# pananananas/MVD

Measured on AMD Instinct MI355X. Metric: UNet forward-passes/sec @512x512 SD2.1+MV adapter, higher is better.
Workload: dtype bf16; 1 GPU; cfg4: configs[3]/[4]: 8 objects x 4 target views per GPU (32 pairs), camera FiLM + cross-view adapter; pairs_per_gpu=32, global_pairs=32, latent=64x64x4, image=512x512, forward=cold, hip_graph=False, q2_statistics=replica-local, parallelism=dp1 (pairs sharded by object), weights=synthetic seeded, SD2.1 shapes (865.9M UNet x2 + 99.2M adapter + 19.1M camera), encoder_weights=distinct

## Files before the change

### include/mvd_hip.h

```cpp
#ifndef MVD_HIP_H
#define MVD_HIP_H
#include <stddef.h>
#include <stdint.h>

#ifdef __cplusplus
extern "C" {
#endif

#define MVD_MAX_LEVELS 4

typedef struct {
  int in_channels;
  int out_channels;
  int num_levels;
  int block_out_channels[MVD_MAX_LEVELS];
  int num_heads[MVD_MAX_LEVELS];
  int layers_per_block;
  int cross_attention_dim;
  int norm_num_groups;
  float norm_eps;
  int cam_output_dim;
  int cam_hidden_dim;
  int simple_cam_encoder;
  float cam_modulation_strength;
// ... 109 lines not shown
int mvd_op_refnorm(const void* x, int batch, int hw, int c, void* y, void* stream);
int mvd_op_refnorm_grouped(const void* x, int batch, int group, int hw, int c, void* y, void* stream);
int mvd_op_film(const void* x, int batch, int hw, int c, const float* scale, const float* shift, void* y, void* stream);
int mvd_op_conv_in(const void* x, int batch, int h, int w, int cin, const float* wt, const float* bias, int cout, void* y,
                   void* stream);
int mvd_op_conv_out(const void* x, int batch, int h, int w, int c, const void* wt, const float* bias, int cout, float* y,
                    void* stream);
int mvd_op_nchw_to_nhwc(const float* x, int batch, int c, int hw, const float* scale, const float* shift, void* y,
                        void* stream);
int mvd_op_nhwc_to_nchw(const void* x, int batch, int hw, int c, float* y, void* stream);
int mvd_op_f32_to_bf16(const float* x, int64_t n, void* y, void* stream);
int mvd_op_skinny_linear(const float* x, int ldx, int batch, int k, const void* w, int wbf16, const float* bias, int n, int act_in,
                         float* y, int ldy, void* stream);
int mvd_gemm_num_configs(void);
int mvd_debug_last_gemm_plan(int* out);
int mvd_debug_last_attention_plan(int* out);
int mvd_debug_last_groupnorm_plan(int* out);
long mvd_debug_up4_launches(void);
int mvd_debug_last_gemm_nowait(void);
int mvd_debug_pick_splitk(int m, int n, int k, int geglu);
int mvd_debug_pick_splitk_conv(int m, int n, int k);
int mvd_gemm_sm_num_tiles(void);
int mvd_debug_set_attention_nw(int nw_log2);
int mvd_debug_ragged_tables(const int* view_counts, int objects, int g, int* adapter, int* text);
int mvd_debug_attention_mapped_grouped(const void* q, const void* k, const void* v, void* o, int batch, int heads, int nq, int nk,
                                       int ldq, int ldk, int ldv, int ldo, float scale, int kv_group, int kv_objects,
                                       const int* kv_index_host, int kv_elements, void* stream);
typedef enum {
  MVD_DBG_NO_SM_LN_FOLD = 1,
  MVD_DBG_SM_NO_SPLITK = 2,
  MVD_DBG_NO_SM = 4,
  MVD_DBG_NO_SPLIT_KV = 8,
  MVD_DBG_ONE_STREAM = 16,
  MVD_DBG_SINGLE_STREAM_POLICY = 32,
  MVD_DBG_SIDE_DEFAULT_PRIORITY = 64,
  MVD_DBG_NO_XS = 128,
  MVD_DBG_NO_WS = 256,
  MVD_DBG_WS_SMALL_MAPS = 512,
  MVD_DBG_WS_BLOCK64 = 1024,
  MVD_DBG_WS_NO_SHORTCUT = 2048,
  MVD_DBG_WS_NOT_IN_ENCODER = 4096,
  MVD_DBG_WS_ONLY_IN_ENCODER = 8192,
  MVD_DBG_WS_THEN_TILED = 16384,
  MVD_DBG_WS_CHECK = 32768,
  MVD_DBG_GRAPH_ONE_STREAM = 65536,
  MVD_DBG_PP_ROW_MAJOR = 131072,
  MVD_DBG_NO_DEEP_CONV_SPLIT = 262144,
  MVD_DBG_LATE_FROM_UP1 = 524288,
  MVD_DBG_NO_UP4 = 1048576,
  MVD_DBG_GN_ONE_PASS = 2097152,
  MVD_DBG_FORK_LATE = 4194304,
  MVD_DBG_SKINNY_VECTOR = 8388608
} mvd_debug_flag_t;
int mvd_debug_set_flags(int flags);

int mvd_op_ddpm_step(const float* model_out, const float* sample, const float* noise, float c0, float c1, float c2,
                     float c3, float sigma, float* out, int64_t n, void* stream);
int mvd_op_cfg_combine(const float* uncond_cond, float guidance_scale, float* out, int64_t n_half, void* stream);
int mvd_op_sampler_step(const float* model_out, int guided, float guidance_scale, const float* sample, const float* x0_prev,
                        const float* noise, float a0, float a1, float p, float q, float r, float sigma, float* out,
                        float* x0_out, int64_t n, void* stream);
int mvd_op_cfg_rescale(const float* uncond_cond, float guidance_scale, float guidance_rescale, float* out, int64_t rows,
                       int64_t n_row, void* stream);
int mvd_op_sampler_step_rescaled(const float* model_out, float guidance_scale, float guidance_rescale, const float* sample,
                                 const float* x0_prev, const float* noise, float a0, float a1, float p, float q, float r,
                                 float sigma, float* out, float* x0_out, int64_t rows, int64_t n_row, void* stream);
int mvd_debug_cfg_rescale_plan(int64_t n_row, int* out);

int mvd_op_freeu(const void* hidden, int C, const void* skip, int Cs, int B, int H, int W, float b, float s, void* hidden_out,
                 void* skip_out, void* stream);

int mvd_op_add_noise(const float* x0, const float* noise, const int32_t* timesteps, const float* sqrt_ac, const float* sqrt_1mac,
                     int num_train_timesteps, float* noisy, float* velocity, int batch, int64_t per_sample, void* stream);
int64_t mvd_op_noise_loss_ws_bytes(int batch, int64_t per_sample);
int mvd_op_noise_loss(const float* pred, const float* noise, const float* x0, const float* noisy, const int32_t* timesteps,
                      const float* sqrt_ac, const float* sqrt_1mac, const float* snr, int num_train_timesteps, int prediction_type,
                      float snr_gamma, float* denoised, float* result, int batch, int64_t per_sample, void* ws, int64_t ws_bytes,
                      void* stream);
int64_t mvd_op_image_metrics_ws_bytes(int n, int c, int h, int w, int want_ssim);
int mvd_op_image_metrics(const float* x, const float* y, int n, int c, int h, int w, float data_range, int want_ssim, float* result,
                         float* per_image, void* ws, int64_t ws_bytes, void* stream);

typedef struct {
  int in_channels;
  int latent_channels;
  int num_levels;
  int block_out_channels[MVD_MAX_LEVELS];
  int layers_per_block;
  int norm_num_groups;
  float norm_eps;
} mvd_vae_config_t;
typedef struct mvd_vae mvd_vae_t;
int mvd_vae_create(const mvd_vae_config_t* cfg, mvd_vae_t** out);
int mvd_vae_destroy(mvd_vae_t* v);
int mvd_vae_set_weight(mvd_vae_t* v, const char* slot, const void* ptr, int64_t numel, int dtype);
int64_t mvd_vae_workspace_bytes(mvd_vae_t* v, int batch, int height, int width, int decode);
int mvd_vae_bind_workspace(mvd_vae_t* v, void* ws, int64_t ws_bytes);
int mvd_vae_encode(mvd_vae_t* v, const float* image_nchw, int batch, int height, int width, float* moments, void* stream);
int mvd_vae_decode(mvd_vae_t* v, const float* latents_nchw, int batch, int height, int width, float* image, void* stream);
int64_t mvd_vae_mid_attention_workspace_bytes(mvd_vae_t* v, int decoder, int batch, int height, int width);
int mvd_vae_mid_attention(mvd_vae_t* v, int decoder, const void* x_nhwc_bf16, int batch, int height, int width, void* out_nhwc_bf16,
                          void* stream);
int mvd_op_softmax_rows(const float* s, int rows, int n, void* p_bf16, void* stream);
int mvd_op_gaussian_sample(const float* moments, const float* noise, int batch, int channels, int hw, float scale, float* out,
                           void* stream);

typedef struct {
// ... 120 lines not shown
```

### mvd_amd/_lib.py

```python
from __future__ import annotations

import ctypes as C
import enum
import os

HERE = os.path.dirname(os.path.abspath(__file__))
LIB_PATH = os.environ.get("MVD_HIP_LIB") or os.path.join(HERE, "libmvd_hip.so")

MVD_MAX_LEVELS = 4
MVD_USE_CAMERA, MVD_USE_IMAGE, MVD_REUSE_REF, MVD_KEEP_FEATURES, MVD_SHARE_REF = 1, 2, 4, 8, 16


class MvdError(RuntimeError):
    pass


class DebugFlag(enum.IntFlag):
    NO_SM_LN_FOLD = 1
    SM_NO_SPLITK = 2
    NO_SM = 4
    NO_SPLIT_KV = 8
    ONE_STREAM = 16
    SINGLE_STREAM_POLICY = 32
    SIDE_DEFAULT_PRIORITY = 64
    NO_XS = 128
    NO_WS = 256
    WS_SMALL_MAPS = 512
    WS_BLOCK64 = 1024
    WS_NO_SHORTCUT = 2048
    WS_NOT_IN_ENCODER = 4096
    WS_ONLY_IN_ENCODER = 8192
    WS_THEN_TILED = 16384
    WS_CHECK = 32768
    GRAPH_ONE_STREAM = 65536
    PP_ROW_MAJOR = 131072
    NO_DEEP_CONV_SPLIT = 262144
    LATE_FROM_UP1 = 524288
    NO_UP4 = 1048576
    GN_ONE_PASS = 2097152
    FORK_LATE = 4194304
    SKINNY_VECTOR = 8388608


class mvd_config_t(C.Structure):
    _fields_ = [
        ("in_channels", C.c_int), ("out_channels", C.c_int), ("num_levels", C.c_int),
        ("block_out_channels", C.c_int * MVD_MAX_LEVELS), ("num_heads", C.c_int * MVD_MAX_LEVELS),
        ("layers_per_block", C.c_int), ("cross_attention_dim", C.c_int), ("norm_num_groups", C.c_int),
        ("norm_eps", C.c_float), ("cam_output_dim", C.c_int), ("cam_hidden_dim", C.c_int),
        ("simple_cam_encoder", C.c_int), ("cam_modulation_strength", C.c_float),
    ]


class mvd_vae_config_t(C.Structure):
    _fields_ = [
        ("in_channels", C.c_int), ("latent_channels", C.c_int), ("num_levels", C.c_int),
        ("block_out_channels", C.c_int * MVD_MAX_LEVELS), ("layers_per_block", C.c_int), ("norm_num_groups", C.c_int),
        ("norm_eps", C.c_float),
    ]


class mvd_text_config_t(C.Structure):
    _fields_ = [
        ("vocab_size", C.c_int), ("hidden_size", C.c_int), ("intermediate_size", C.c_int), ("num_layers", C.c_int),
        ("num_heads", C.c_int), ("max_positions", C.c_int), ("layer_norm_eps", C.c_float), ("act", C.c_int),
    ]


class mvd_vision_config_t(C.Structure):
    _fields_ = [
        ("image_size", C.c_int), ("patch_size", C.c_int), ("hidden_size", C.c_int), ("intermediate_size", C.c_int),
        ("num_layers", C.c_int), ("num_heads", C.c_int), ("projection_dim", C.c_int), ("layer_norm_eps", C.c_float), ("act", C.c_int),
    ]


class mvd_forward_args_t(C.Structure):
    _fields_ = [
        ("batch", C.c_int), ("height", C.c_int), ("width", C.c_int), ("text_len", C.c_int),
        ("sample", C.c_void_p), ("timesteps", C.c_void_p), ("text", C.c_void_p),
        ("source_camera", C.c_void_p), ("target_camera", C.c_void_p), ("cam_rows", C.c_int), ("cam_batch", C.c_int),
        ("fourier_proj", C.c_void_p), ("source_latents", C.c_void_p), ("encoder_text", C.c_void_p),
        ("ref_batch", C.c_int), ("flags", C.c_int), ("out", C.c_void_p), ("views", C.c_int),
    ]


_SIGS = {
    "mvd_last_error": (C.c_char_p, []),
    "mvd_engine_create": (C.c_int, [C.POINTER(mvd_config_t), C.POINTER(C.c_void_p)]),
    "mvd_engine_destroy": (C.c_int, [C.c_void_p]),
    "mvd_engine_set_weight": (C.c_int, [C.c_void_p, C.c_int, C.c_char_p, C.c_void_p, C.c_int64, C.c_int]),
    "mvd_engine_clear_weights": (C.c_int, [C.c_void_p, C.c_int]),
    "mvd_engine_workspace_bytes": (C.c_int64, [C.c_void_p, C.c_int, C.c_int, C.c_int, C.c_int, C.c_int]),
    "mvd_engine_workspace_bytes_args": (C.c_int64, [C.c_void_p, C.POINTER(mvd_forward_args_t)]),
    "mvd_engine_workspace_bytes_objects": (C.c_int64, [C.c_void_p, C.POINTER(mvd_forward_args_t), C.c_int]),
# ... 21 lines not shown
    "mvd_engine_get_camera_embedding": (C.c_int, [C.c_void_p, C.c_void_p, C.c_void_p]),
    "mvd_op_linear": (C.c_int, [C.c_void_p, C.c_void_p, C.c_int, C.c_int, C.c_void_p, C.c_void_p, C.c_void_p, C.c_int,
                                C.c_int, C.c_void_p, C.c_float, C.c_int, C.c_void_p, C.c_int, C.c_int, C.c_int, C.c_int,
                                C.c_int, C.c_void_p, C.c_void_p]),
    "mvd_op_ln_linear": (C.c_int, [C.c_void_p, C.c_int, C.c_void_p, C.c_void_p, C.c_void_p, C.c_float, C.c_int, C.c_void_p,
                                   C.c_int, C.c_int, C.c_void_p]),
    "mvd_op_linear_xs": (C.c_int, [C.c_void_p, C.c_int, C.c_void_p, C.c_int, C.c_int, C.c_int, C.c_int, C.c_int, C.c_float,
                                   C.c_void_p, C.c_int, C.c_void_p, C.c_int, C.c_int, C.c_void_p]),
    "mvd_op_conv3x3_ws": (C.c_int, [C.c_void_p, C.c_int, C.c_int, C.c_int, C.c_int, C.c_void_p, C.c_void_p, C.c_void_p, C.c_int,
                                    C.c_void_p, C.c_void_p, C.c_void_p, C.c_int, C.c_int, C.c_void_p, C.c_int, C.c_int, C.c_void_p]),
    "mvd_op_conv3x3": (C.c_int, [C.c_void_p, C.c_int, C.c_int, C.c_int, C.c_int, C.c_int, C.c_int, C.c_int, C.c_void_p, C.c_void_p,
                                 C.c_void_p, C.c_int, C.c_void_p, C.c_void_p, C.c_void_p, C.c_int, C.c_int, C.c_void_p,
                                 C.c_int, C.c_int, C.c_int, C.c_void_p, C.c_void_p]),
    "mvd_op_attention": (C.c_int, [C.c_void_p, C.c_void_p, C.c_void_p, C.c_void_p, C.c_int, C.c_int, C.c_int, C.c_int,
                                   C.c_int, C.c_int, C.c_int, C.c_int, C.c_float, C.c_void_p]),
    "mvd_op_attention_grouped": (C.c_int, [C.c_void_p, C.c_void_p, C.c_void_p, C.c_void_p, C.c_int, C.c_int, C.c_int, C.c_int,
                                           C.c_int, C.c_int, C.c_int, C.c_int, C.c_float, C.c_int, C.c_void_p]),
    "mvd_op_attention_objects": (C.c_int, [C.c_void_p, C.c_void_p, C.c_void_p, C.c_void_p, C.c_int, C.c_int, C.c_int, C.c_int,
                                           C.c_int, C.c_int, C.c_int, C.c_int, C.c_float, C.c_int, C.c_int, C.c_void_p]),
    "mvd_op_attention_mapped": (C.c_int, [C.c_void_p, C.c_void_p, C.c_void_p, C.c_void_p, C.c_int, C.c_int, C.c_int, C.c_int,
                                          C.c_int, C.c_int, C.c_int, C.c_int, C.c_float, C.POINTER(C.c_int), C.c_int, C.c_void_p]),
    "mvd_debug_attention_mapped_grouped": (C.c_int, [C.c_void_p, C.c_void_p, C.c_void_p, C.c_void_p, C.c_int, C.c_int, C.c_int, C.c_int,
                                                     C.c_int, C.c_int, C.c_int, C.c_int, C.c_float, C.c_int, C.c_int, C.POINTER(C.c_int),
                                                     C.c_int, C.c_void_p]),
    "mvd_op_attention_split_ws_bytes": (C.c_int64, [C.c_int, C.c_int, C.c_int, C.c_int]),
    "mvd_op_attention_split": (C.c_int, [C.c_void_p, C.c_void_p, C.c_void_p, C.c_void_p, C.c_int, C.c_int, C.c_int, C.c_int, C.c_int,
                                         C.c_int, C.c_int, C.c_int, C.c_int, C.c_void_p, C.c_void_p]),
    "mvd_op_groupnorm": (C.c_int, [C.c_void_p, C.c_void_p, C.c_int, C.c_int, C.c_int, C.c_int, C.c_int, C.c_float,
                                   C.c_void_p, C.c_void_p, C.c_int, C.c_void_p, C.c_void_p, C.c_void_p]),
    "mvd_op_layernorm": (C.c_int, [C.c_void_p, C.c_int, C.c_int, C.c_float, C.c_void_p, C.c_void_p, C.c_void_p, C.c_void_p]),
    "mvd_op_refnorm": (C.c_int, [C.c_void_p, C.c_int, C.c_int, C.c_int, C.c_void_p, C.c_void_p]),
    "mvd_op_refnorm_grouped": (C.c_int, [C.c_void_p, C.c_int, C.c_int, C.c_int, C.c_int, C.c_void_p, C.c_void_p]),
    "mvd_op_film": (C.c_int, [C.c_void_p, C.c_int, C.c_int, C.c_int, C.c_void_p, C.c_void_p, C.c_void_p, C.c_void_p]),
    "mvd_op_conv_in": (C.c_int, [C.c_void_p, C.c_int, C.c_int, C.c_int, C.c_int, C.c_void_p, C.c_void_p, C.c_int, C.c_void_p, C.c_void_p]),
    "mvd_op_conv_out": (C.c_int, [C.c_void_p, C.c_int, C.c_int, C.c_int, C.c_int, C.c_void_p, C.c_void_p, C.c_int, C.c_void_p, C.c_void_p]),
    "mvd_op_nchw_to_nhwc": (C.c_int, [C.c_void_p, C.c_int, C.c_int, C.c_int, C.c_void_p, C.c_void_p, C.c_void_p, C.c_void_p]),
    "mvd_op_nhwc_to_nchw": (C.c_int, [C.c_void_p, C.c_int, C.c_int, C.c_int, C.c_void_p, C.c_void_p]),
    "mvd_op_f32_to_bf16": (C.c_int, [C.c_void_p, C.c_int64, C.c_void_p, C.c_void_p]),
    "mvd_op_skinny_linear": (C.c_int, [C.c_void_p, C.c_int, C.c_int, C.c_int, C.c_void_p, C.c_int, C.c_void_p, C.c_int, C.c_int,
                                        C.c_void_p, C.c_int, C.c_void_p]),
    "mvd_gemm_num_configs": (C.c_int, []),
    "mvd_debug_last_gemm_plan": (C.c_int, [C.POINTER(C.c_int)]),
    "mvd_debug_up4_launches": (C.c_long, []),
    "mvd_op_conv3x3_up4": (C.c_int, [C.c_void_p, C.c_int, C.c_int, C.c_int, C.c_int, C.c_void_p, C.c_void_p, C.c_void_p, C.c_int, C.c_int,
                                     C.c_void_p]),
    "mvd_debug_last_gemm_nowait": (C.c_int, []),
    "mvd_debug_last_attention_plan": (C.c_int, [C.POINTER(C.c_int)]),
    "mvd_debug_last_groupnorm_plan": (C.c_int, [C.POINTER(C.c_int)]),
    "mvd_debug_pick_splitk": (C.c_int, [C.c_int, C.c_int, C.c_int, C.c_int]),
    "mvd_debug_pick_splitk_conv": (C.c_int, [C.c_int, C.c_int, C.c_int]),
    "mvd_gemm_sm_num_tiles": (C.c_int, []),
    "mvd_debug_set_attention_nw": (C.c_int, [C.c_int]),
    "mvd_debug_set_flags": (C.c_int, [C.c_int]),
    "mvd_op_ddpm_step": (C.c_int, [C.c_void_p, C.c_void_p, C.c_void_p, C.c_float, C.c_float, C.c_float, C.c_float,
                                   C.c_float, C.c_void_p, C.c_int64, C.c_void_p]),
    "mvd_op_cfg_combine": (C.c_int, [C.c_void_p, C.c_float, C.c_void_p, C.c_int64, C.c_void_p]),
    "mvd_op_sampler_step": (C.c_int, [C.c_void_p, C.c_int, C.c_float, C.c_void_p, C.c_void_p, C.c_void_p, C.c_float, C.c_float,
                                      C.c_float, C.c_float, C.c_float, C.c_float, C.c_void_p, C.c_void_p, C.c_int64, C.c_void_p]),
    "mvd_op_cfg_rescale": (C.c_int, [C.c_void_p, C.c_float, C.c_float, C.c_void_p, C.c_int64, C.c_int64, C.c_void_p]),
    "mvd_op_sampler_step_rescaled": (C.c_int, [C.c_void_p, C.c_float, C.c_float, C.c_void_p, C.c_void_p, C.c_void_p, C.c_float,
                                               C.c_float, C.c_float, C.c_float, C.c_float, C.c_float, C.c_void_p, C.c_void_p,
                                               C.c_int64, C.c_int64, C.c_void_p]),
    "mvd_debug_cfg_rescale_plan": (C.c_int, [C.c_int64, C.POINTER(C.c_int)]),
    "mvd_engine_set_freeu": (C.c_int, [C.c_void_p, C.c_float, C.c_float, C.c_float, C.c_float]),
    "mvd_engine_clear_freeu": (C.c_int, [C.c_void_p]),
    "mvd_op_freeu": (C.c_int, [C.c_void_p, C.c_int, C.c_void_p, C.c_int, C.c_int, C.c_int, C.c_int, C.c_float, C.c_float, C.c_void_p,
                               C.c_void_p, C.c_void_p]),
    "mvd_op_add_noise": (C.c_int, [C.c_void_p, C.c_void_p, C.c_void_p, C.c_void_p, C.c_void_p, C.c_int, C.c_void_p, C.c_void_p, C.c_int,
                                   C.c_int64, C.c_void_p]),
    "mvd_op_noise_loss_ws_bytes": (C.c_int64, [C.c_int, C.c_int64]),
    "mvd_op_noise_loss": (C.c_int, [C.c_void_p, C.c_void_p, C.c_void_p, C.c_void_p, C.c_void_p, C.c_void_p, C.c_void_p, C.c_void_p,
                                    C.c_int, C.c_int, C.c_float, C.c_void_p, C.c_void_p, C.c_int, C.c_int64, C.c_void_p, C.c_int64,
                                    C.c_void_p]),
    "mvd_op_image_metrics_ws_bytes": (C.c_int64, [C.c_int, C.c_int, C.c_int, C.c_int, C.c_int]),
    "mvd_op_image_metrics": (C.c_int, [C.c_void_p, C.c_void_p, C.c_int, C.c_int, C.c_int, C.c_int, C.c_float, C.c_int, C.c_void_p,
                                       C.c_void_p, C.c_void_p, C.c_int64, C.c_void_p]),
    "mvd_vae_create": (C.c_int, [C.POINTER(mvd_vae_config_t), C.POINTER(C.c_void_p)]),
    "mvd_vae_destroy": (C.c_int, [C.c_void_p]),
    "mvd_vae_set_weight": (C.c_int, [C.c_void_p, C.c_char_p, C.c_void_p, C.c_int64, C.c_int]),
    "mvd_vae_workspace_bytes": (C.c_int64, [C.c_void_p, C.c_int, C.c_int, C.c_int, C.c_int]),
    "mvd_vae_bind_workspace": (C.c_int, [C.c_void_p, C.c_void_p, C.c_int64]),
    "mvd_vae_encode": (C.c_int, [C.c_void_p, C.c_void_p, C.c_int, C.c_int, C.c_int, C.c_void_p, C.c_void_p]),
    "mvd_vae_decode": (C.c_int, [C.c_void_p, C.c_void_p, C.c_int, C.c_int, C.c_int, C.c_void_p, C.c_void_p]),
    "mvd_vae_mid_attention_workspace_bytes": (C.c_int64, [C.c_void_p, C.c_int, C.c_int, C.c_int, C.c_int]),
    "mvd_vae_mid_attention": (C.c_int, [C.c_void_p, C.c_int, C.c_void_p, C.c_int, C.c_int, C.c_int, C.c_void_p, C.c_void_p]),
    "mvd_op_softmax_rows": (C.c_int, [C.c_void_p, C.c_int, C.c_int, C.c_void_p, C.c_void_p]),
    "mvd_op_gaussian_sample": (C.c_int, [C.c_void_p, C.c_void_p, C.c_int, C.c_int, C.c_int, C.c_float, C.c_void_p, C.c_void_p]),
    "mvd_text_create": (C.c_int, [C.POINTER(mvd_text_config_t), C.POINTER(C.c_void_p)]),
    "mvd_text_destroy": (C.c_int, [C.c_void_p]),
    "mvd_text_set_weight": (C.c_int, [C.c_void_p, C.c_char_p, C.c_void_p, C.c_int64, C.c_int]),
    "mvd_text_workspace_bytes": (C.c_int64, [C.c_void_p, C.c_int, C.c_int]),
    "mvd_text_bind_workspace": (C.c_int, [C.c_void_p, C.c_void_p, C.c_int64]),
    "mvd_text_encode": (C.c_int, [C.c_void_p, C.c_void_p, C.c_int, C.c_int, C.c_void_p, C.c_void_p]),
    "mvd_op_attention_causal": (C.c_int, [C.c_void_p, C.c_void_p, C.c_void_p, C.c_void_p, C.c_int, C.c_int, C.c_int, C.c_int,
                                          C.c_int, C.c_int, C.c_int, C.c_float, C.c_void_p]),
    "mvd_vision_create": (C.c_int, [C.POINTER(mvd_vision_config_t), C.POINTER(C.c_void_p)]),
    "mvd_vision_destroy": (C.c_int, [C.c_void_p]),
    "mvd_vision_set_weight": (C.c_int, [C.c_void_p, C.c_char_p, C.c_void_p, C.c_int64, C.c_int]),
    "mvd_vision_workspace_bytes": (C.c_int64, [C.c_void_p, C.c_int, C.c_int, C.c_int, C.c_int]),
    "mvd_vision_bind_workspace": (C.c_int, [C.c_void_p, C.c_void_p, C.c_int64]),
    "mvd_vision_preprocess": (C.c_int, [C.c_void_p, C.c_void_p, C.c_int, C.c_int, C.c_int, C.c_int, C.c_int, C.c_int,
                                        C.POINTER(C.c_float), C.POINTER(C.c_float), C.c_int, C.c_void_p, C.c_void_p]),
    "mvd_vision_patch_rows_offset": (C.c_int64, [C.c_void_p]),
    "mvd_vision_encode": (C.c_int, [C.c_void_p, C.c_void_p, C.c_int, C.c_void_p, C.c_void_p, C.c_void_p, C.c_void_p]),
    "mvd_op_clip_pool_project": (C.c_int, [C.c_void_p, C.c_void_p, C.c_void_p, C.c_int, C.c_int, C.c_int, C.c_int, C.c_void_p,
                                           C.c_void_p, C.c_float, C.c_void_p, C.c_int, C.c_void_p, C.c_void_p, C.c_void_p]),
# ... 146 lines not shown
```

### mvd_amd/csrc/misc.hip

```cpp
#include <stdarg.h>
#include <stdio.h>
#include <stdlib.h>
#include "host_util.h"

static thread_local char g_err[512] = "";
void mvd_set_error(const char* fmt, ...) {
  va_list ap;
  va_start(ap, fmt);
  vsnprintf(g_err, sizeof(g_err), fmt, ap);
  va_end(ap);
}
extern "C" const char* mvd_last_error(void) { return g_err; }

namespace {

__global__ void nchw_to_nhwc_kernel(const float* __restrict__ x, int c, int hw, const float* __restrict__ scale,
                                    const float* __restrict__ shift, int ld_ss, bf16_t* __restrict__ y, long total) {
  const long i = (long)blockIdx.x * blockDim.x + threadIdx.x;
  if (i >= total) return;
  const int ch = i % c;
  const long bp = i / c;
  const int p = bp % hw;
  const int b = bp / hw;
  float v = x[((size_t)b * c + ch) * hw + p];
  if (scale) v = v * scale[(size_t)b * ld_ss + ch] + shift[(size_t)b * ld_ss + ch];
  y[i] = f2bf(v);
}

__global__ void nhwc_to_nchw_f32_kernel(const bf16_t* __restrict__ x, int hw, int c, float* __restrict__ y, long total) {
  const long i = (long)blockIdx.x * blockDim.x + threadIdx.x;
  if (i >= total) return;
  const int p = i % hw;
  const long bc = i / hw;
  const int ch = bc % c;
  const int b = bc / c;
  y[i] = bf2f(x[((size_t)b * hw + p) * c + ch]);
}

__global__ void film_kernel(const bf16_t* __restrict__ x, int hw, int c, const float* __restrict__ scale,
                            const float* __restrict__ shift, int ld_ss, bf16_t* __restrict__ y, long nvec) {
  const int vec = c >> 3;
  for (long e = (long)blockIdx.x * blockDim.x + threadIdx.x; e < nvec; e += (long)gridDim.x * blockDim.x) {
    const int v = e % vec;
    const long bp = e / vec;
    const int b = bp / hw;
    const u32x4 in = *reinterpret_cast<const u32x4*>(x + e * 8);
    const float* sc = scale + (size_t)b * ld_ss + v * 8;
    const float* sf = shift + (size_t)b * ld_ss + v * 8;
    u32x4 o;
#pragma unroll
    for (int j = 0; j < 4; ++j)
      o[j] = pack2bf(fmaf(bflo(in[j]), sc[2 * j], sf[2 * j]), fmaf(bfhi(in[j]), sc[2 * j + 1], sf[2 * j + 1]));
    *reinterpret_cast<u32x4*>(y + e * 8) = o;
  }
}

__global__ void conv_in_kernel(const bf16_t* __restrict__ x, int h, int w, int cin, const float* __restrict__ wt,
                               const float* __restrict__ bias, int cout, bf16_t* __restrict__ y, long total) {
// ... 10 lines not shown
#pragma unroll
  for (int j = 0; j < 8; ++j) acc[j] = bias[g * 8 + j];
  for (int tap = 0; tap < 9; ++tap) {
    const int iy = oy + tap / 3 - 1, ix = ox + tap % 3 - 1;
    if ((unsigned)iy >= (unsigned)h || (unsigned)ix >= (unsigned)w) continue;
    const bf16_t* xp = x + ((size_t)b * hw + iy * w + ix) * cin;
    for (int ci = 0; ci < cin; ++ci) {
      const float xv = bf2f(xp[ci]);
#pragma unroll
      for (int j = 0; j < 8; ++j) acc[j] = fmaf(xv, wt[((size_t)(g * 8 + j) * 9 + tap) * cin + ci], acc[j]);
    }
  }
  u32x4 o = {pack2bf(acc[0], acc[1]), pack2bf(acc[2], acc[3]), pack2bf(acc[4], acc[5]), pack2bf(acc[6], acc[7])};
  *reinterpret_cast<u32x4*>(y + bp * cout + g * 8) = o;
}

__global__ __launch_bounds__(256) void conv_out_kernel(const bf16_t* __restrict__ x, int batch, int h, int w, int c,
                                                        const bf16_t* __restrict__ wt, const float* __restrict__ bias,
                                                        int cout, float* __restrict__ y) {
  const int lane = threadIdx.x & 63;
  const long pix = (long)blockIdx.x * 4 + (threadIdx.x >> 6);
  const int hw = h * w;
  if (pix >= (long)batch * hw) return;
  const int b = pix / hw, p = pix % hw;
  const int oy = p / w, ox = p % w;
  const int vec = c >> 3;
  float acc[8];
#pragma unroll
  for (int j = 0; j < 8; ++j) acc[j] = 0.f;
  for (int q = lane; q < 9 * vec; q += 64) {
    const int tap = q / vec, v = q % vec;
    const int iy = oy + tap / 3 - 1, ix = ox + tap % 3 - 1;
    if ((unsigned)iy >= (unsigned)h || (unsigned)ix >= (unsigned)w) continue;
    const u32x4 xv = *reinterpret_cast<const u32x4*>(x + ((size_t)b * hw + iy * w + ix) * c + v * 8);
#pragma unroll
    for (int co = 0; co < 8; ++co) {
      if (co < cout) {
        const u32x4 wv = *reinterpret_cast<const u32x4*>(wt + ((size_t)co * 9 + tap) * c + v * 8);
        float a = acc[co];
#pragma unroll
        for (int j = 0; j < 4; ++j) {
          a = fmaf(bflo(xv[j]), bflo(wv[j]), a);
          a = fmaf(bfhi(xv[j]), bfhi(wv[j]), a);
        }
        acc[co] = a;
      }
    }
  }
#pragma unroll
  for (int co = 0; co < 8; ++co) {
    if (co < cout) {
      const float t = wave_sum(acc[co]);
      if (lane == 0) y[((size_t)b * cout + co) * hw + p] = t + bias[co];
    }
  }
}

__global__ void f32_to_bf16_kernel(const float* __restrict__ x, long n, bf16_t* __restrict__ y) {
  for (long i = (long)blockIdx.x * blockDim.x + threadIdx.x; i < n; i += (long)gridDim.x * blockDim.x) y[i] = f2bf(x[i]);
}

template <bool WBF16>
__global__ __launch_bounds__(256) void skinny_linear_kernel(const float* __restrict__ x, int ldx, int batch, int k,
                                                             const void* __restrict__ wv, const float* __restrict__ bias,
                                                             int n, int act_in, float* __restrict__ y, int ldy) {
  constexpr int BC = 32;
  const int lane = threadIdx.x & 63;
  const int o = blockIdx.x * 4 + (threadIdx.x >> 6);
  if (o >= n) return;
  const bool vec = !WBF16 && (k & 3) == 0 && (ldx & 3) == 0;
  for (int b0 = 0; b0 < batch; b0 += BC) {
    float acc[BC];
#pragma unroll
    for (int j = 0; j < BC; ++j) acc[j] = 0.f;
    if (vec) {
      const float* wr = reinterpret_cast<const float*>(wv) + (size_t)o * k;
      for (int kk = lane * 4; kk < k; kk += 256) {
        const f32x4 w4 = *reinterpret_cast<const f32x4*>(wr + kk);
#pragma unroll
        for (int j = 0; j < BC; ++j) {
          if (b0 + j < batch) {
            f32x4 x4 = *reinterpret_cast<const f32x4*>(x + (size_t)(b0 + j) * ldx + kk);
            if (act_in == 1) { x4[0] = silu_f(x4[0]); x4[1] = silu_f(x4[1]); x4[2] = silu_f(x4[2]); x4[3] = silu_f(x4[3]); }
            acc[j] = fmaf(x4[0], w4[0], fmaf(x4[1], w4[1], fmaf(x4[2], w4[2], fmaf(x4[3], w4[3], acc[j]))));
          }
        }
      }
    } else {
      for (int kk = lane; kk < k; kk += 64) {
        float wgt;
        if (WBF16) wgt = bf2f(reinterpret_cast<const bf16_t*>(wv)[(size_t)o * k + kk]);
        else wgt = reinterpret_cast<const float*>(wv)[(size_t)o * k + kk];
#pragma unroll
        for (int j = 0; j < BC; ++j) {
          if (b0 + j < batch) {
            float xv = x[(size_t)(b0 + j) * ldx + kk];
            if (act_in == 1) xv = silu_f(xv);
            acc[j] = fmaf(xv, wgt, acc[j]);
          }
        }
      }
    }
#pragma unroll
    for (int j = 0; j < BC; ++j) {
      if (b0 + j < batch) {
        const float t = wave_sum(acc[j]);
// ... 279 lines not shown
  for (long i = (long)blockIdx.x * blockDim.x + threadIdx.x; i < n; i += (long)gridDim.x * blockDim.x) {
    const float va = a[i], vb = b[i], vr = r[i];
    if (__float_as_uint(va) != __float_as_uint(vb)) { __hip_atomic_fetch_add(cnt, 1ull, __ATOMIC_RELAXED, __HIP_MEMORY_SCOPE_SYSTEM); __hip_atomic_store(cnt + 3, (unsigned long long)i, __ATOMIC_RELAXED, __HIP_MEMORY_SCOPE_SYSTEM); }
    if (!(fabsf(va - vr) <= tol)) __hip_atomic_fetch_add(cnt + 1, 1ull, __ATOMIC_RELAXED, __HIP_MEMORY_SCOPE_SYSTEM);
    if (!(fabsf(vb - vr) <= tol)) __hip_atomic_fetch_add(cnt + 2, 1ull, __ATOMIC_RELAXED, __HIP_MEMORY_SCOPE_SYSTEM);
  }
}
#endif

int mvd_launch_conv_out(const bf16_t* x, int batch, int h, int w, int c, const bf16_t* wt, const float* bias, int cout,
                        float* y, hipStream_t s) {
  if (!x || !y || !wt || !bias || batch <= 0 || h <= 0 || w <= 0 || (c % 8) || cout <= 0 || cout > 8) { mvd_set_error("conv_out: bad arguments"); return -1; }
#ifdef MVD_PROBE
  if (MVD_ENV_INT("MVD_CONV_OUT4", 0)) {
    const long quads = (long)batch * h * ((w + 3) / 4);
    hipLaunchKernelGGL(conv_out4_kernel, dim3(nblk(quads, 4)), dim3(256), 0, s, x, batch, h, w, c, wt, bias, cout, y);
    if (MVD_ENV_INT("MVD_CONV_OUT_HASH", 0)) {
      static unsigned long long* dsum = nullptr; static float* y1 = nullptr; static size_t y1n = 0;
      const size_t on = (size_t)batch * cout * h * w;
      if (!dsum) (void)hipMalloc(&dsum, 3 * sizeof(unsigned long long));
      if (y1n < on) { if (y1) (void)hipFree(y1); (void)hipMalloc(&y1, on * sizeof(float)); y1n = on; }
      (void)hipMemsetAsync(dsum, 0, 3 * sizeof(unsigned long long), s);
      const long pix1 = (long)batch * h * w;
      hipLaunchKernelGGL(conv_out_kernel, dim3(nblk(pix1, 4)), dim3(256), 0, s, x, batch, h, w, c, wt, bias, cout, y1);
      hipLaunchKernelGGL(word_sum_kernel, dim3(1024), dim3(256), 0, s, reinterpret_cast<const unsigned*>(x), (long)((size_t)batch * h * w * c / 2), dsum);
      hipLaunchKernelGGL(word_sum_kernel, dim3(1024), dim3(256), 0, s, reinterpret_cast<const unsigned*>(y), (long)on, dsum + 1);
      hipLaunchKernelGGL(word_sum_kernel, dim3(1024), dim3(256), 0, s, reinterpret_cast<const unsigned*>(y1), (long)on, dsum + 2);
      unsigned long long hs[3] = {0, 0, 0};
      (void)hipMemcpyAsync(hs, dsum, sizeof(hs), hipMemcpyDeviceToHost, s);
      (void)hipStreamSynchronize(s);
      fprintf(stderr, "conv_out hash pid %d: input %016llx  out(4-pixel) %016llx  out(1-pixel, same input) %016llx\n", (int)getpid(), hs[0], hs[1], hs[2]);
    }
    if (MVD_ENV_INT("MVD_CONV_OUT_CMP", 0)) {
      static unsigned long long* cnt = nullptr; static float* yb = nullptr; static float* yr = nullptr; static size_t yn = 0;
      static unsigned long long seen[3] = {0, 0, 0}; static int calls = 0;
      const size_t on = (size_t)batch * cout * h * w;
      if (!cnt) { (void)hipHostMalloc(&cnt, 4 * sizeof(unsigned long long), hipHostMallocMapped); cnt[0] = cnt[1] = cnt[2] = cnt[3] = 0; }
      if (yn < on) { if (yb) { (void)hipFree(yb); (void)hipFree(yr); } (void)hipMalloc(&yb, on * sizeof(float)); (void)hipMalloc(&yr, on * sizeof(float)); yn = on; }
      hipLaunchKernelGGL(conv_out4_kernel, dim3(nblk(quads, 4)), dim3(256), 0, s, x, batch, h, w, c, wt, bias, cout, yb);
      hipLaunchKernelGGL(conv_out_kernel, dim3(nblk((long)batch * h * w, 4)), dim3(256), 0, s, x, batch, h, w, c, wt, bias, cout, yr);
      hipLaunchKernelGGL(conv_out_cmp_kernel, dim3(256), dim3(256), 0, s, y, yb, yr, (long)on, 1e-3f, cnt);
      ++calls;
      volatile unsigned long long* vc = cnt;
      const unsigned long long c0 = vc[0], c1 = vc[1], c2 = vc[2];
      if (c0 != seen[0] || c1 != seen[1] || c2 != seen[2] || calls == 2 || calls == 20) {
        seen[0] = c0; seen[1] = c1; seen[2] = c2;
        fprintf(stderr, "conv_out cmp pid %d after ~%d calls: first!=second %llu  |first-ref|>1e-3 %llu  |second-ref|>1e-3 %llu  last idx %llu (x mod 4 = %llu)\n",
                (int)getpid(), calls - 1, c0, c1, c2, (unsigned long long)vc[3], (unsigned long long)vc[3] % 4);
      }
    }
    return launch_check("conv_out4");
  }
#endif
  const long pix = (long)batch * h * w;
  hipLaunchKernelGGL(conv_out_kernel, dim3(nblk(pix, 4)), dim3(256), 0, s, x, batch, h, w, c, wt, bias, cout, y);
  return launch_check("conv_out");
}

int mvd_launch_f32_to_bf16(const float* x, int64_t n, bf16_t* y, hipStream_t s) {
  if (!x || !y || n <= 0) { mvd_set_error("f32_to_bf16: bad arguments"); return -1; }
  int grid = nblk(n, 256);
  if (grid > 4096) grid = 4096;
  hipLaunchKernelGGL(f32_to_bf16_kernel, dim3(grid), dim3(256), 0, s, x, (long)n, y);
  return launch_check("f32_to_bf16");
}

int mvd_launch_skinny_linear(const float* x, int ldx, int batch, int k, const void* w, int wbf16, const float* bias, int n,
                             int act_in, float* y, int ldy, hipStream_t s) {
  if (!x || !w || !y || batch <= 0 || batch > 4096 || k <= 0 || n <= 0 || ldx < k || ldy < n) { mvd_set_error("skinny_linear: bad arguments"); return -1; }
  const int kv = wbf16 ? 8 : 4;
  const bool vec = (k % kv) == 0 && (ldx % 4) == 0 && (((uintptr_t)x | (uintptr_t)w) & 15) == 0;
  static const int use_vec = MVD_ENV_INT("MVD_SKINNY_VEC", 1);
  if (vec && batch >= 8 && !(mvd_debug_flags() & MVD_DBG_SKINNY_VECTOR)) {
    const MvdSegTable none{};
    if (wbf16) hipLaunchKernelGGL((skinny_mfma_kernel<true, false>), dim3(nblk(n, 32)), dim3(256), 0, s, x, ldx, batch, k, w, bias, n, act_in, y, ldy, none, 0);
    else hipLaunchKernelGGL((skinny_mfma_kernel<false, false>), dim3(nblk(n, 32)), dim3(256), 0, s, x, ldx, batch, k, w, bias, n, act_in, y, ldy, none, 0);
    return launch_check("skinny_mfma");
  }
  if (vec && use_vec) {
    constexpr int F = 2;
    const dim3 g(nblk(n, 4 * F));
    if (wbf16) hipLaunchKernelGGL((skinny_linear_vec_kernel<true, F>), g, dim3(256), 0, s, x, ldx, batch, k, w, bias, n, act_in, y, ldy);
    else hipLaunchKernelGGL((skinny_linear_vec_kernel<false, F>), g, dim3(256), 0, s, x, ldx, batch, k, w, bias, n, act_in, y, ldy);
    return launch_check("skinny_linear");
  }
  if (wbf16) hipLaunchKernelGGL(skinny_linear_kernel<true>, dim3(nblk(n, 4)), dim3(256), 0, s, x, ldx, batch, k, w, bias, n, act_in, y, ldy);
  else hipLaunchKernelGGL(skinny_linear_kernel<false>, dim3(nblk(n, 4)), dim3(256), 0, s, x, ldx, batch, k, w, bias, n, act_in, y, ldy);
  return launch_check("skinny_linear");
}

int mvd_launch_skinny_linear_grouped(const float* x, int ldx, int xseg, int batch, int k, const float* w, const float* bias, int n,
                                     const MvdSegTable& seg, float* y, int ldy, hipStream_t s) {
  if (!x || !w || !y || batch <= 0 || batch > 4096 || k <= 0 || (k % 4) || (ldx % 4) || n <= 0 || ldy < n || seg.n < 1 || seg.n > 16 ||
      seg.end[seg.n - 1] != n || (((uintptr_t)x | (uintptr_t)w) & 15) || (xseg % 4)) { mvd_set_error("skinny_linear_grouped: bad arguments"); return -1; }
  for (int g = 0; g < seg.n; ++g) if (seg.end[g] % 2) { mvd_set_error("skinny_linear_grouped: segment ends must be even"); return -1; }
  bool tiles_ok = batch >= 8 && !(mvd_debug_flags() & MVD_DBG_SKINNY_VECTOR);
  for (int g = 0; g + 1 < seg.n; ++g) tiles_ok = tiles_ok && seg.end[g] % 32 == 0;
  if (tiles_ok) {
    hipLaunchKernelGGL((skinny_mfma_kernel<false, true>), dim3(nblk(n, 32)), dim3(256), 0, s, x, ldx, batch, k, (const void*)w, bias, n, 0, y, ldy, seg, xseg);
    return launch_check("skinny_mfma_grouped");
  }
  hipLaunchKernelGGL((skinny_linear_vec_kernel<false, 2, true>), dim3(nblk(n, 8)), dim3(256), 0, s, x, ldx, batch, k, (const void*)w, bias, n, 0, y, ldy, seg, xseg);
  return launch_check("skinny_linear_grouped");
}

__global__ void film_params_grouped_kernel(const float* __restrict__ raw, int batch, int ldraw, const MvdSegTable seg, float strength,
                                           float* __restrict__ out, int out_rows, int total) {
  const int i = blockIdx.x * blockDim.x + threadIdx.x;
  if (i >= total) return;
  const int half = seg.end[seg.n - 1] / 2;
// ... 67 lines not shown
```

### mvd_amd/ops.py

```python
from __future__ import annotations

import ctypes as C
from typing import Optional

import torch

from . import _lib as L


def _p(t: Optional[torch.Tensor]):
    if t is None:
        return None
    assert t.is_cuda and t.is_contiguous(), "ops expect contiguous CUDA tensors"
    return C.c_void_p(t.data_ptr())


_s = L.stream


def _bf16(*ts):
    for t in ts:
        if t is not None:
            assert t.dtype == torch.bfloat16, "expected bf16"

# ... 231 lines not shown
        ws = torch.empty(need, dtype=torch.uint8, device=f_real.device)
    out = torch.empty(subsets, dtype=torch.float64, device=f_real.device)
    sums = torch.empty(subsets, 3, dtype=torch.float64, device=f_real.device) if want_sums else None
    L.call("mvd_op_kid_mmd", _p(f_real), f_real.shape[0], _p(f_fake), f_fake.shape[0], d, _p(idx), subsets, m, int(degree),
           float(1.0 / d if gamma is None else gamma), float(coef), _p(ws), need, _p(sums), _p(out), _s())
    return (out, sums) if want_sums else out


def fc_logits(f, w):
    assert f.dtype == torch.float32 and w.dtype == torch.float32 and f.dim() == 2 and w.dim() == 2 and f.shape[1] == w.shape[1]
    out = torch.empty(f.shape[0], w.shape[0], dtype=torch.float32, device=f.device)
    L.call("mvd_op_fc_logits", _p(f), f.shape[0], f.shape[1], _p(w), w.shape[0], _p(out), _s())
    return out


def inception_score_chunks(logits, perm, splits):
    assert logits.dtype == torch.float32 and logits.dim() == 2 and perm.dtype == torch.int32 and perm.shape == (logits.shape[0],)
    n, classes = logits.shape
    need = L.lib().mvd_op_inception_score_workspace_bytes(n, classes, int(splits))
    if need < 0:
        raise L.MvdError(f"mvd_op_inception_score_workspace_bytes: {L.last_error()}")
    ws = torch.empty(need, dtype=torch.uint8, device=logits.device)
    out = torch.empty(min(int(splits), n), dtype=torch.float64, device=logits.device)
    chunks = C.c_int(0)
    L.call("mvd_op_inception_score", _p(logits), n, classes, _p(perm), int(splits), _p(ws), need, _p(out), C.byref(chunks), _s())
    return out[:chunks.value]


def knn_radii(f, k, force_parts=0, want_list=False, ws=None):
    assert f.dtype == torch.float32 and f.dim() == 2
    n, d = f.shape
    need = L.lib().mvd_op_knn_radii_workspace_bytes(n, int(k), int(force_parts))
    if need < 0:
        raise L.MvdError(f"mvd_op_knn_radii_workspace_bytes: {L.last_error()}")
    if ws is None:
        ws = torch.empty(need, dtype=torch.uint8, device=f.device)
    radii = torch.empty(n, dtype=torch.float64, device=f.device)
    knn = torch.empty(n, int(k) + 1, dtype=torch.float64, device=f.device) if want_list else None
    L.call("mvd_op_knn_radii", _p(f), n, d, int(k), int(force_parts), _p(radii), _p(knn), _p(ws), need, _s())
    return (radii, knn) if want_list else radii


def manifold_counts(q, r, radii_sq, closed, want_query=True, want_ref=True):
    assert q.dtype == torch.float32 and r.dtype == torch.float32 and q.dim() == 2 and r.dim() == 2 and q.shape[1] == r.shape[1]
    assert radii_sq.dtype == torch.float64 and radii_sq.shape == (r.shape[0],)
    hq = torch.empty(q.shape[0], dtype=torch.int32, device=q.device) if want_query else None
    hr = torch.empty(r.shape[0], dtype=torch.int32, device=q.device) if want_ref else None
    L.call("mvd_op_manifold_counts", _p(q), q.shape[0], _p(r), r.shape[0], q.shape[1], _p(radii_sq), int(bool(closed)), _p(hq), _p(hr), _s())
    return hq, hr


def up4_launches() -> int:
    return int(L.lib().mvd_debug_up4_launches())


def attention(q, k, v, heads, scale=0.125):
    _bf16(q, k, v)
    B, nq, _ = q.shape
    nk = k.shape[1]
    assert q.stride(2) == 1 and k.stride(2) == 1 and v.stride(2) == 1
    assert q.stride(0) == nq * q.stride(1) and k.stride(0) == nk * k.stride(1) and v.stride(0) == nk * v.stride(1)
    out = torch.empty(B, nq, heads * 64, device=q.device, dtype=torch.bfloat16)
    L.call("mvd_op_attention", C.c_void_p(q.data_ptr()), C.c_void_p(k.data_ptr()), C.c_void_p(v.data_ptr()), _p(out),
           B, heads, nq, nk, q.stride(1), k.stride(1), v.stride(1), heads * 64, float(scale), _s())
    return out


def attention_grouped(q, k, v, heads, kv_group, scale=0.125):
    _bf16(q, k, v)
    B, nq, _ = q.shape
    nk = k.shape[1]
    assert kv_group >= 1 and B % kv_group == 0 and k.shape[0] == B // kv_group and v.shape[0] == B // kv_group, (B, kv_group, k.shape, v.shape)
    assert q.stride(2) == 1 and k.stride(2) == 1 and v.stride(2) == 1
    assert q.stride(0) == nq * q.stride(1) and k.stride(0) == nk * k.stride(1) and v.stride(0) == nk * v.stride(1)
    out = torch.empty(B, nq, heads * 64, device=q.device, dtype=torch.bfloat16)
    L.call("mvd_op_attention_grouped", C.c_void_p(q.data_ptr()), C.c_void_p(k.data_ptr()), C.c_void_p(v.data_ptr()), _p(out),
           B, heads, nq, nk, q.stride(1), k.stride(1), v.stride(1), heads * 64, float(scale), int(kv_group), _s())
    return out


def attention_objects(q, k, v, heads, kv_group, kv_objects, scale=0.125):
    _bf16(q, k, v)
    B, nq, _ = q.shape
    nk = k.shape[1]
    kvg = max(int(kv_group), 1)
    assert kv_objects >= 0 and B % (kvg * max(int(kv_objects), 1)) == 0 and k.shape[0] == B // kvg and v.shape[0] == B // kvg, (B, kv_group, kv_objects, k.shape, v.shape)
    assert q.stride(2) == 1 and k.stride(2) == 1 and v.stride(2) == 1
    assert q.stride(0) == nq * q.stride(1) and k.stride(0) == nk * k.stride(1) and v.stride(0) == nk * v.stride(1)
    out = torch.empty(B, nq, heads * 64, device=q.device, dtype=torch.bfloat16)
    L.call("mvd_op_attention_objects", C.c_void_p(q.data_ptr()), C.c_void_p(k.data_ptr()), C.c_void_p(v.data_ptr()), _p(out),
           B, heads, nq, nk, q.stride(1), k.stride(1), v.stride(1), heads * 64, float(scale), int(kv_group), int(kv_objects), _s())
    return out


def attention_mapped(q, k, v, heads, kv_index, scale=0.125):
    _bf16(q, k, v)
    B, nq, _ = q.shape
    nk = k.shape[1]
    idx = [int(i) for i in (kv_index.tolist() if isinstance(kv_index, torch.Tensor) else kv_index)]
    if isinstance(kv_index, torch.Tensor):
        assert not kv_index.is_cuda and not kv_index.is_floating_point(), "kv_index: a CPU int tensor"
    assert len(idx) == B and k.shape[0] == v.shape[0], (B, len(idx), k.shape, v.shape)
    assert q.stride(2) == 1 and k.stride(2) == 1 and v.stride(2) == 1
    assert q.stride(0) == nq * q.stride(1) and k.stride(0) == nk * k.stride(1) and v.stride(0) == nk * v.stride(1)
    out = torch.empty(B, nq, heads * 64, device=q.device, dtype=torch.bfloat16)
    L.call("mvd_op_attention_mapped", C.c_void_p(q.data_ptr()), C.c_void_p(k.data_ptr()), C.c_void_p(v.data_ptr()), _p(out),
# ... 309 lines not shown
```

Before: 535.7 forward-passes/s.

## Add MFMA implicit-GEMM kernel for the final 3x3 output convolution

Replaces the wave-reduction conv_out kernel with an MFMA-based implicit GEMM. The full 3x3 weight tensor is staged in LDS, padded to 16 output columns, and activations are read through buffer loads with out-of-bounds masking for the image borders. Each wave computes a 16-pixel strip over T rows, with T chosen from the row count. The intent is to cut the cost of the small-Cout final conv, which the scalar dot-product kernel handles poorly. In exchange it wastes MFMA lanes on padded output channels, needs large dynamic LDS, and keeps the old kernel behind a debug flag as a fallback.

```diff
diff --git a/include/mvd_hip.h b/include/mvd_hip.h
--- a/include/mvd_hip.h
+++ b/include/mvd_hip.h
@@ -185,7 +185,11 @@
   MVD_DBG_FORK_LATE = 4194304,
   MVD_DBG_SKINNY_VECTOR = 8388608
 } mvd_debug_flag_t;
+typedef enum {
+  MVD_DBG_CONV_OUT_VECTOR = 16777216
+} mvd_debug_tail_flag_t;
 int mvd_debug_set_flags(int flags);
+int mvd_debug_last_conv_out_form(void);
 
 int mvd_op_ddpm_step(const float* model_out, const float* sample, const float* noise, float c0, float c1, float c2,
                      float c3, float sigma, float* out, int64_t n, void* stream);
diff --git a/mvd_amd/_lib.py b/mvd_amd/_lib.py
--- a/mvd_amd/_lib.py
+++ b/mvd_amd/_lib.py
@@ -40,6 +40,10 @@
     GN_ONE_PASS = 2097152
     FORK_LATE = 4194304
     SKINNY_VECTOR = 8388608
+
+
+class TailDebugFlag(enum.IntFlag):
+    CONV_OUT_VECTOR = 16777216
 
 
 class mvd_config_t(C.Structure):
@@ -167,6 +171,7 @@
     "mvd_gemm_sm_num_tiles": (C.c_int, []),
     "mvd_debug_set_attention_nw": (C.c_int, [C.c_int]),
     "mvd_debug_set_flags": (C.c_int, [C.c_int]),
+    "mvd_debug_last_conv_out_form": (C.c_int, []),
     "mvd_op_ddpm_step": (C.c_int, [C.c_void_p, C.c_void_p, C.c_void_p, C.c_float, C.c_float, C.c_float, C.c_float,
                                    C.c_float, C.c_void_p, C.c_int64, C.c_void_p]),
     "mvd_op_cfg_combine": (C.c_int, [C.c_void_p, C.c_float, C.c_void_p, C.c_int64, C.c_void_p]),
diff --git a/mvd_amd/csrc/misc.hip b/mvd_amd/csrc/misc.hip
--- a/mvd_amd/csrc/misc.hip
+++ b/mvd_amd/csrc/misc.hip
@@ -1,9 +1,11 @@
 #include <stdarg.h>
 #include <stdio.h>
 #include <stdlib.h>
+#include "bufaddr.h"
 #include "host_util.h"
 
 static thread_local char g_err[512] = "";
+static thread_local int g_conv_out_form = -1;
 void mvd_set_error(const char* fmt, ...) {
   va_list ap;
   va_start(ap, fmt);
@@ -120,6 +122,87 @@
     if (co < cout) {
       const float t = wave_sum(acc[co]);
       if (lane == 0) y[((size_t)b * cout + co) * hw + p] = t + bias[co];
+    }
+  }
+}
+
+template <int T>
+__global__ __launch_bounds__(256) void conv_out_mfma_kernel(const bf16_t* __restrict__ x, int h, int w, int c,
+                                                             const bf16_t* __restrict__ wt, const float* __restrict__ bias,
+                                                             int cout, float* __restrict__ y, int nyb, int nxt, int njobs) {
+  extern __shared__ __attribute__((aligned(16))) unsigned char co_lds[];
+  const int cs = c >> 5;
+  const int K = 9 * c;
+  constexpr int SB = 6;
+  const int nchunk = 9 * cs * 32;
+  for (int i0 = threadIdx.x; i0 < nchunk; i0 += 256 * SB) {
+    u32x4 v[SB];
+#pragma unroll
+    for (int u = 0; u < SB; ++u) {
+      const int i = i0 + u * 256 < nchunk ? i0 + u * 256 : nchunk - 1;
+      const int col = (i & 7) < cout ? (i & 7) : cout - 1, kq = i >> 3;
+      v[u] = *reinterpret_cast<const u32x4*>(wt + (size_t)col * K + kq * 8);
+    }
+#pragma unroll
+    for (int u = 0; u < SB; ++u) {
+      const int i = i0 + u * 256;
+      if (i < nchunk) *reinterpret_cast<u32x4*>(co_lds + i * 16) = (i & 7) < cout ? v[u] : u32x4{0u, 0u, 0u, 0u};
+    }
+  }
+  __syncthreads();
+  const int lane = threadIdx.x & 63, r = lane & 15, q = lane >> 4;
+  const int job = __builtin_amdgcn_readfirstlane(blockIdx.x * 4 + (threadIdx.x >> 6));
+  if (job >= njobs) return;
+  const int xt = job % nxt, yb = (job / nxt) % nyb, b = job / (nxt * nyb);
+  const int x0 = xt * 16, y0 = yb * T;
+  const size_t img = (size_t)h * w * c;
+  const __amdgpu_buffer_rsrc_t rs = buf_rsrc(x + (size_t)b * img - c, (int)((img + c) * 2));
+  const unsigned char* bl = co_lds + q * 128 + (r & 7) * 16;
+  const unsigned m_left = x0 + r - 1 < 0 ? OOB : 0u, m_right = x0 + r + 1 >= w ? OOB : 0u;
+  constexpr int D = T == 1 ? 15 : T == 2 ? 10 : 6;
+  const int nf = 3 * cs;
+  f32x4 acc[T];
+#pragma unroll
+  for (int t = 0; t < T; ++t) acc[t] = f32x4{0.f, 0.f, 0.f, 0.f};
+#pragma unroll
+  for (int yi = 0; yi < T + 2; ++yi) {
+    const int yy = y0 - 1 + yi;
+    if (yy < 0 || yy >= h) continue;
+    const unsigned base = (unsigned)(((yy * w + x0 + r) * c + q * 8) * 2);
+    auto load = [&](int f) {
+      const unsigned v = base | (m_left & (f < cs ? ~0u : 0u)) | (m_right & (f >= 2 * cs ? ~0u : 0u)) | (f >= nf ? OOB : 0u);
+      return __builtin_amdgcn_raw_buffer_load_b128(rs, (int)v, f * 64, 0);
+    };
+    u32x4 A[D];
+#pragma unroll
+    for (int u = 0; u < D; ++u) A[u] = load(u);
+    for (int f0 = 0; f0 < nf; f0 += D) {
+#pragma unroll
+      for (int u = 0; u < D; ++u) {
+        const int f = f0 + u, fb = f < nf ? f : nf - 1;
+#pragma unroll
+        for (int dy = 0; dy < 3; ++dy) {
+          const int t = yi - dy;
+          if (t >= 0 && t < T) {
+            const bf16x8 wf = *reinterpret_cast<const bf16x8*>(bl + (dy * nf + fb) * 512);
+            acc[t] = __builtin_amdgcn_mfma_f32_16x16x32_bf16(__builtin_bit_cast(bf16x8, A[u]), wf, acc[t], 0, 0, 0);
+          }
+        }
+        A[u] = load(f + D);
+      }
+    }
+  }
+  if (r < cout) {
+    const float bv = bias[r];
+    const size_t hw = (size_t)h * w;
+#pragma unroll
+    for (int t = 0; t < T; ++t) {
+      if (y0 + t < h) {
+        f32x4 o = acc[t];
+#pragma unroll
+        for (int i = 0; i < 4; ++i) o[i] += bv;
+        *reinterpret_cast<f32x4*>(y + ((size_t)b * cout + r) * hw + (size_t)(y0 + t) * w + x0 + q * 4) = o;
+      }
     }
   }
 }
@@ -505,10 +588,34 @@
     return launch_check("conv_out4");
   }
 #endif
+  const size_t img_bytes = (size_t)(h * (size_t)w + 1) * c * 2;
+  const size_t lds = (size_t)9 * (c / 32) * 512;
+  if (c % 32 == 0 && w % 16 == 0 && img_bytes < OOB && lds <= 160 * 1024 && !((uintptr_t)y & 15) &&
+      !(mvd_debug_flags() & MVD_DBG_CONV_OUT_VECTOR)) {
+    const int nxt = w / 16;
+    const long rows = (long)batch * h * nxt;
+    const int T = rows >= 4 * 1024 ? 4 : rows >= 2 * 1024 ? 2 : 1;
+    const int nyb = (h + T - 1) / T;
+    const long njobs = (long)batch * nyb * nxt;
+    if (njobs < (1L << 30)) {
+      const unsigned grid = (unsigned)nblk(njobs, 4);
+      auto* k = T == 4 ? &conv_out_mfma_kernel<4> : T == 2 ? &conv_out_mfma_kernel<2> : &conv_out_mfma_kernel<1>;
+      if (lds > 65536) {
+        hipError_t e = hipFuncSetAttribute(reinterpret_cast<const void*>(k), hipFuncAttributeMaxDynamicSharedMemorySize, (int)lds);
+        if (e != hipSuccess) { mvd_set_error("conv_out: hipFuncSetAttribute: %s", hipGetErrorString(e)); return -2; }
+      }
+      hipLaunchKernelGGL(k, dim3(grid), dim3(256), lds, s, x, h, w, c, wt, bias, cout, y, nyb, nxt, (int)njobs);
+      g_conv_out_form = 1;
+      return launch_check("conv_out_mfma");
+    }
+  }
   const long pix = (long)batch * h * w;
   hipLaunchKernelGGL(conv_out_kernel, dim3(nblk(pix, 4)), dim3(256), 0, s, x, batch, h, w, c, wt, bias, cout, y);
+  g_conv_out_form = 0;
   return launch_check("conv_out");
 }
+
+extern "C" int mvd_debug_last_conv_out_form(void) { return g_conv_out_form; }
 
 int mvd_launch_f32_to_bf16(const float* x, int64_t n, bf16_t* y, hipStream_t s) {
   if (!x || !y || n <= 0) { mvd_set_error("f32_to_bf16: bad arguments"); return -1; }
diff --git a/mvd_amd/ops.py b/mvd_amd/ops.py
--- a/mvd_amd/ops.py
+++ b/mvd_amd/ops.py
@@ -307,6 +307,10 @@
 
 def up4_launches() -> int:
     return int(L.lib().mvd_debug_up4_launches())
+
+
+def last_conv_out_form() -> int:
+    return int(L.lib().mvd_debug_last_conv_out_form())
 
 
 def attention(q, k, v, heads, scale=0.125):
```

Measured after the change: 537.2 forward-passes/s (median of 6 runs). About the same (+0.3%).
